# AronCao49/MoPA

Hardware: AMD Instinct MI355X
Metric: scans/sec (joint 2D+3D train step) at 1/2/4/8 MI355X; sparse-conv HBM GB/s (higher is better)
Workload: dtype f32

## Files before the change

mopa_amd/csrc/wino4c9.hip:

```cpp
#include "wino4.h"
#include <stdlib.h>
#include <stdio.h>

typedef float f32x16c __attribute__((ext_vector_type(16)));
typedef float f32x4c __attribute__((ext_vector_type(4)));

#define C9_TM 32
#define C9_CN 64
#define C9_KC 16
#define C9_PITCH 34

struct C9Args {
  const float* in; const float* Uq; const float* bias; float* out; const float* stats;
  int ld_in, ld_out, B, H, W, th, tw, T, Cin, Cout, accumulate, imgs_per_group, bn_c0, nco;
  long long* prof;
};

__device__ __forceinline__ void c9_bt(float d0, float d1, float d2, float d3, float d4, float d5, float& t0, float& t1, float& t2, float& t3,
                                      float& t4, float& t5) {
  t0 = fmaf(4.f, d0, fmaf(-5.f, d2, d4));
  const float p = fmaf(-4.f, d2, d4), q = fmaf(-4.f, d1, d3);
  t1 = p + q;
  t2 = p - q;
  const float r = d4 - d2, s = d3 - d1;
  t3 = fmaf(2.f, s, r);
  t4 = fmaf(-2.f, s, r);
  t5 = fmaf(4.f, d1, fmaf(-5.f, d3, d5));
}

template <bool BN>
__global__ __launch_bounds__(512, 2) void k_wino4_conv9(const C9Args a) {
  __shared__ __attribute__((aligned(16))) float c9_lds[36 * C9_KC * C9_PITCH + 36 * 512];
  float* const Vs = c9_lds;
  float* const Ps = c9_lds + 36 * C9_KC * C9_PITCH;
  const int t = threadIdx.x, lane = t & 63, wv = __builtin_amdgcn_readfirstlane(t >> 6);
  const int nco = a.nco;
  const int grp = blockIdx.x / (8 * nco), r8 = blockIdx.x - grp * 8 * nco;
  const int cob = r8 >> 3, tg = grp * 8 + (r8 & 7);
  const int t0 = tg * C9_TM;
  if (t0 >= a.T) return;
  const int co0 = cob * C9_CN;
  const int H = a.H, W = a.W, tw = a.tw, thw = a.th * a.tw;
#ifdef C9_PROFILE
  long long pt[8] = {0, 0, 0, 0, 0, 0, 0, 0}, tprev = __builtin_readcyclecounter();
#define C9_T(K_) { const long long n_ = __builtin_readcyclecounter(); pt[K_] += n_ - tprev; tprev = n_; }
#else
#define C9_T(K_)
#endif

  const int ts = t >> 4, ch = t & 15;
  const int tile = t0 + ts;
  const bool tv = tile < a.T;
  const int tb = tile / thw, rt = tile - tb * thw, ty = rt / tw, tx = rt - ty * tw;
  const int ab = tv ? tb : 0, ay = tv ? ty : 0, ax = tv ? tx : 0;
  const uint32_t ld4 = (uint32_t)a.ld_in * 4u;
  unsigned okm = 0;
  uint32_t cof[6];
#pragma unroll
  for (int i = 0; i < 6; ++i) {
    okm |= (tv && (unsigned)(4 * ay - 1 + i) < (unsigned)H ? 1u : 0u) << i;
    okm |= ((unsigned)(4 * ax - 1 + i) < (unsigned)W ? 1u : 0u) << (8 + i);
    cof[i] = (uint32_t)min(max(4 * ax - 1 + i, 0), W - 1) * ld4 + (uint32_t)ch * 4u;
  }
  const int abH = ab * H, y0 = 4 * ay - 1;
  const bool interior = __all(tv && ty >= 1 && tx >= 1 && 4 * ty + 4 < H && 4 * tx + 4 < W) != 0;
  const char* __restrict__ inb = reinterpret_cast<const char*>(a.in);
  float* __restrict__ vw = Vs + ch * C9_PITCH + ts;
  float sc = 1.f, sh = 0.f;
  bool bn_ch = false;

  const int l32 = lane & 31, lk = lane >> 5, g = wv & 3, coh = wv >> 2;
  const int pa0 = 3 * (g >> 1), pb0 = 3 * (g & 1);
  const int nci = a.Cin / C9_KC;
  const int64_t pstride = (int64_t)a.Cin * a.Cout;
  const int nco32 = a.Cout / 32;
  const char* __restrict__ ub = reinterpret_cast<const char*>(a.Uq + (int64_t)(pa0 * 6 + pb0) * pstride + (int64_t)(cob * 2 + coh) * 512);
  const uint32_t ul = (uint32_t)lane * 16u;

  f32x16c acc[9];
#pragma unroll
  for (int q = 0; q < 9; ++q)
#pragma unroll
    for (int e = 0; e < 16; ++e) acc[q][e] = 0.f;

  auto row_off = [&](const int i) -> uint32_t { return (uint32_t)((abH + min(max(y0 + i, 0), H - 1)) * W) * ld4; };
  const unsigned ps0 = (unsigned)(uintptr_t)(__attribute__((address_space(3))) void*)&Ps[0] + (unsigned)wv * 256u;
  auto patch_dma = [&](const int n, const uint32_t cb) {
    __builtin_amdgcn_global_load_lds((const __attribute__((address_space(1))) void*)(inb + (row_off(n / 6) + cof[n % 6] + cb)),
                                     (__attribute__((address_space(3))) void*)(uintptr_t)(ps0 + (unsigned)n * 2048u), 4, 0, 0);
  };
  auto patch_bn = [&](int cib) {
    if (BN) {
      const int c_ = cib * C9_KC + ch;
      bn_ch = c_ >= a.bn_c0;
      if (bn_ch) {
        const float* __restrict__ sg = a.stats + (int64_t)((tv ? tb : 0) / a.imgs_per_group) * 4 * (a.Cin - a.bn_c0) + (c_ - a.bn_c0);
        sc = sg[0];
        sh = sg[a.Cin - a.bn_c0];
      }
    }
  };
#pragma unroll
  for (int n = 0; n < 36; ++n) patch_dma(n, 0u);
  patch_bn(0);
  const unsigned vr_b = (unsigned)(uintptr_t)(__attribute__((address_space(3))) void*)&Vs[0] +
                        (unsigned)(((pa0 * 6 + pb0) * C9_KC + lk) * C9_PITCH + l32) * 4u;

  for (int cib = 0; cib < nci; ++cib) {
    C9_T(0)
    {
      __builtin_amdgcn_s_waitcnt(0x0F70);
      float d[36];
#pragma unroll
      for (int n = 0; n < 36; ++n) d[n] = Ps[n * 512 + t];
      if (BN || !interior) {
#pragma unroll
        for (int n = 0; n < 36; ++n) {
          float v = d[n];
          if (BN) {
            const float o = fmaf(v, sc, sh);
            v = bn_ch ? (o > 0.f ? o : o * 0.f) : v;
          }
          d[n] = ((okm >> (n / 6)) & (okm >> (8 + n % 6)) & 1u) ? v : 0.f;
        }
      }
      C9_T(1)
      float m[6][6];
#pragma unroll
      for (int j = 0; j < 6; ++j)
        c9_bt(d[j], d[6 + j], d[12 + j], d[18 + j], d[24 + j], d[30 + j], m[0][j], m[1][j], m[2][j], m[3][j], m[4][j], m[5][j]);
#pragma unroll
      for (int i = 0; i < 6; ++i) {
        float v[6];
        c9_bt(m[i][0], m[i][1], m[i][2], m[i][3], m[i][4], m[i][5], v[0], v[1], v[2], v[3], v[4], v[5]);
#pragma unroll
        for (int j = 0; j < 6; ++j) vw[((i * 6 + j) * C9_KC) * C9_PITCH] = v[j];
      }
    }
    C9_T(2)
    __syncthreads();
    C9_T(3)
    {
      const bool more = cib + 1 < nci;
      const uint32_t cb = (uint32_t)((more ? cib + 1 : cib) * C9_KC) * 4u;
      const char* __restrict__ up = ub + (int64_t)cib * nco32 * 2048;
      f32x4c b0, b1, n0, n1;
#define C9_WLOAD(X0, X1, PTR) \
  asm volatile("global_load_dwordx4 %0, %2, %3\n\tglobal_load_dwordx4 %1, %2, %3 offset:1024" : "=&v"(X0), "=&v"(X1) : "v"(ul), "s"(PTR))
#define C9_WWAIT(N, X0, X1) asm volatile("s_waitcnt vmcnt(" #N ")" : "+v"(X0), "+v"(X1))
      C9_WLOAD(b0, b1, up);
#pragma unroll
      for (int q = 0; q < 9; ++q) {
        if (q + 1 < 9) {
          const char* __restrict__ un = up + (int64_t)(((q + 1) / 3) * 6 + (q + 1) % 3) * pstride * 4;
          if (q & 1) { C9_WLOAD(b0, b1, un); } else { C9_WLOAD(n0, n1, un); }
        }
        float av[8];
#define C9_OFF(KK) "i"((((q / 3) * 6 + q % 3) * C9_KC + 2 * (KK)) * C9_PITCH * 4)
        asm volatile("ds_read_b32 %0, %8 offset:%9\n\tds_read_b32 %1, %8 offset:%10\n\tds_read_b32 %2, %8 offset:%11\n\tds_read_b32 %3, %8 offset:%12\n\t"
                     "ds_read_b32 %4, %8 offset:%13\n\tds_read_b32 %5, %8 offset:%14\n\tds_read_b32 %6, %8 offset:%15\n\tds_read_b32 %7, %8 offset:%16\n\t"
                     "s_waitcnt lgkmcnt(0)"
                     : "=&v"(av[0]), "=&v"(av[1]), "=&v"(av[2]), "=&v"(av[3]), "=&v"(av[4]), "=&v"(av[5]), "=&v"(av[6]), "=&v"(av[7])
                     : "v"(vr_b), C9_OFF(0), C9_OFF(1), C9_OFF(2), C9_OFF(3), C9_OFF(4), C9_OFF(5), C9_OFF(6), C9_OFF(7));
        if (q & 1) {
          if (q == 7) { C9_WWAIT(2, n0, n1); } else { C9_WWAIT(8, n0, n1); }
#pragma unroll
          for (int kk = 0; kk < 4; ++kk) acc[q] = __builtin_amdgcn_mfma_f32_32x32x2f32(av[kk], n0[kk], acc[q], 0, 0, 0);
#pragma unroll
          for (int kk = 0; kk < 4; ++kk) acc[q] = __builtin_amdgcn_mfma_f32_32x32x2f32(av[4 + kk], n1[kk], acc[q], 0, 0, 0);
        } else {
          if (q == 0) { C9_WWAIT(2, b0, b1); } else if (q == 8) { C9_WWAIT(0, b0, b1); } else { C9_WWAIT(8, b0, b1); }
#pragma unroll
          for (int kk = 0; kk < 4; ++kk) acc[q] = __builtin_amdgcn_mfma_f32_32x32x2f32(av[kk], b0[kk], acc[q], 0, 0, 0);
#pragma unroll
          for (int kk = 0; kk < 4; ++kk) acc[q] = __builtin_amdgcn_mfma_f32_32x32x2f32(av[4 + kk], b1[kk], acc[q], 0, 0, 0);
        }
        if (q < 6) {
#pragma unroll
          for (int n = 6 * q; n < 6 * q + 6; ++n) patch_dma(n, cb);
        }
      }
      if (more) patch_bn(cib + 1);
    }
    C9_T(4)
    __builtin_amdgcn_s_barrier();
    C9_T(5)
  }

  constexpr float AT[4][6] = {{1.f, 1.f, 1.f, 1.f, 1.f, 0.f}, {0.f, 1.f, -1.f, 2.f, -2.f, 0.f}, {0.f, 1.f, 1.f, 4.f, 4.f, 0.f},
                              {0.f, 1.f, -1.f, 8.f, -8.f, 1.f}};
  float ar_[4][3];
#pragma unroll
  for (int i = 0; i < 4; ++i)
#pragma unroll
    for (int k = 0; k < 3; ++k) ar_[i][k] = (g >> 1) ? AT[i][3 + k] : AT[i][k];
  __builtin_amdgcn_s_waitcnt(0x0F70);
  __syncthreads();
  float* __restrict__ tsb = c9_lds;
  const int stl = t0 + (t >> 4), sq = (t & 15) * 4;
  const f32x4c bv = a.bias ? *reinterpret_cast<const f32x4c*>(a.bias + co0 + sq) : (f32x4c){0.f, 0.f, 0.f, 0.f};
  const int sb_ = stl / thw, sr_ = stl - sb_ * thw, sty = sr_ / tw, stx = sr_ - sty * tw;
  float* __restrict__ obase = a.out + ((int64_t)(sb_ * H + 4 * sty) * W + 4 * stx) * a.ld_out + co0 + sq;
  for (int i = 0; i < 4; ++i) {
#pragma unroll
    for (int e = 0; e < 16; ++e) {
      const int til = 8 * (e >> 2) + 4 * lk + (e & 3);
#pragma unroll
      for (int b = 0; b < 3; ++b) {
        const float tv_ = fmaf(ar_[i][0], acc[b][e], fmaf(ar_[i][1], acc[3 + b][e], ar_[i][2] * acc[6 + b][e]));
        tsb[(((g >> 1) * 6 + pb0 + b) * C9_TM + til) * C9_CN + coh * 32 + l32] = tv_;
      }
    }
    __syncthreads();
    {
      f32x4c tt[6];
#pragma unroll
      for (int b = 0; b < 6; ++b) {
        const f32x4c u0 = *reinterpret_cast<const f32x4c*>(tsb + (b * C9_TM + (t >> 4)) * C9_CN + sq);
        const f32x4c u1 = *reinterpret_cast<const f32x4c*>(tsb + ((6 + b) * C9_TM + (t >> 4)) * C9_CN + sq);
        tt[b] = u0 + u1;
      }
      if (stl < a.T && 4 * sty + i < H) {
        float* __restrict__ o = obase + (int64_t)i * W * a.ld_out;
#pragma unroll
        for (int j = 0; j < 4; ++j) {
          f32x4c y = bv;
#pragma unroll
          for (int b = 0; b < 6; ++b)
            if (AT[j][b] != 0.f) y += AT[j][b] * tt[b];
          if (4 * stx + j < W) {
            f32x4c* __restrict__ op = reinterpret_cast<f32x4c*>(o + (int64_t)j * a.ld_out);
            *op = a.accumulate ? *op + y : y;
          }
        }
      }
    }
    __syncthreads();
  }
#ifdef C9_PROFILE
  C9_T(6)
  if (blockIdx.x == 100 && t == 0)
    for (int k = 0; k < 8; ++k) a.prof[k] = pt[k];
#endif
}


MOPA_API int mopa_wino4_conv9(const float* in, int32_t ld_in, const float* Uq, const float* bias, float* out, int32_t ld_out, int32_t B, int32_t H,
                              int32_t W, int32_t Cin, int32_t Cout, int32_t accumulate, const float* stats, int32_t n_groups, int32_t bn_c0,
                              void* stream) {
  if (B <= 0 || H <= 0 || W <= 0 || Cin <= 0 || Cout <= 0 || Cin % C9_KC || Cout % C9_CN || ld_in < Cin || ld_out < Cout ||
      ((uintptr_t)Uq & 15) || ((uintptr_t)out & 15) || (ld_out & 3) || ((uintptr_t)bias & 15) || !in || !Uq || !out)
    return MOPA_ERR_ARG;
  if (stats && (n_groups < 1 || B % n_groups || bn_c0 < 0 || bn_c0 >= Cin)) return MOPA_ERR_ARG;
  if ((int64_t)B * H * W * ld_in >= (1ll << 30) || (int64_t)B * H * W * ld_out >= (1ll << 31)) return MOPA_ERR_ARG;
  C9Args a;
  a.in = in; a.Uq = Uq; a.bias = bias; a.out = out; a.stats = stats;
  a.ld_in = ld_in; a.ld_out = ld_out; a.B = B; a.H = H; a.W = W; a.th = (H + 3) / 4; a.tw = (W + 3) / 4;
  const int64_t T = (int64_t)B * a.th * a.tw;
  if (T >= (1 << 30)) return MOPA_ERR_ARG;
  a.T = (int)T; a.Cin = Cin; a.Cout = Cout; a.accumulate = accumulate;
  a.imgs_per_group = stats ? B / n_groups : 1;
  a.bn_c0 = stats ? bn_c0 : 0;
  a.nco = Cout / C9_CN;
  a.prof = nullptr;
  const int64_t ntg = (cdiv64(T, C9_TM) + 7) / 8 * 8;
  const int64_t nblk = ntg * a.nco;
  if (nblk >= (1ll << 31)) return MOPA_ERR_ARG;
#ifdef C9_PROFILE
  static long long* prof = nullptr;
  if (!prof) hipMallocManaged(&prof, 128);
  a.prof = prof;
#endif
  if (stats) k_wino4_conv9<true><<<(unsigned)nblk, 512, 0, (hipStream_t)stream>>>(a);
  else k_wino4_conv9<false><<<(unsigned)nblk, 512, 0, (hipStream_t)stream>>>(a);
  MOPA_CHECK_LAUNCH();
#ifdef C9_PROFILE
  hipStreamSynchronize((hipStream_t)stream);
  {
    const double n_ = Cin / C9_KC;
    printf("[c9 profile] block 100 wave 0, cycles per step: loop head %.0f | patch loads + apply %.0f | transform + lds stores %.0f | barrier %.0f | "
           "multiply %.0f | barrier %.0f | output transform + exchange + store (per item) %.0f   (steps per item %.0f)\n",
           prof[0] / n_, prof[1] / n_, prof[2] / n_, prof[3] / n_, prof[4] / n_, prof[5] / n_, (double)prof[6], n_);
  }
#endif
  return MOPA_OK;
}
```

Before: 424.0.

## Use 16-byte global-to-LDS DMA for Winograd input patches when aligned

Adds a WIDE variant of the F(4x4,3x3) Winograd conv kernel. It loads each input patch with 9 global_load_lds dwordx4 transfers per wave instead of 36 scalar dword ones, with precomputed per-lane gather offsets built via shuffles. The LDS patch layout becomes wave-major to match, and the vmcnt waits and DMA issue points inside the multiply loop are rescheduled for the smaller DMA count. The host picks WIDE when the input is 16-byte aligned and ld_in is a multiple of 4. The aim is fewer memory instructions and better coalescing, at the cost of more template instances and extra address setup.

```diff
diff --git a/mopa_amd/csrc/wino4c9.hip b/mopa_amd/csrc/wino4c9.hip
--- a/mopa_amd/csrc/wino4c9.hip
+++ b/mopa_amd/csrc/wino4c9.hip
@@ -28,7 +28,7 @@
   t5 = fmaf(4.f, d1, fmaf(-5.f, d3, d5));
 }
 
-template <bool BN>
+template <bool BN, bool WIDE>
 __global__ __launch_bounds__(512, 2) void k_wino4_conv9(const C9Args a) {
   __shared__ __attribute__((aligned(16))) float c9_lds[36 * C9_KC * C9_PITCH + 36 * 512];
   float* const Vs = c9_lds;
@@ -43,6 +43,7 @@
   const int H = a.H, W = a.W, tw = a.tw, thw = a.th * a.tw;
 #ifdef C9_PROFILE
   long long pt[8] = {0, 0, 0, 0, 0, 0, 0, 0}, tprev = __builtin_readcyclecounter();
+  const long long tstart = tprev;
 #define C9_T(K_) { const long long n_ = __builtin_readcyclecounter(); pt[K_] += n_ - tprev; tprev = n_; }
 #else
 #define C9_T(K_)
@@ -55,14 +56,23 @@
   const int ab = tv ? tb : 0, ay = tv ? ty : 0, ax = tv ? tx : 0;
   const uint32_t ld4 = (uint32_t)a.ld_in * 4u;
   unsigned okm = 0;
-  uint32_t cof[6];
+  uint32_t cof[WIDE ? 9 : 6];
 #pragma unroll
   for (int i = 0; i < 6; ++i) {
     okm |= (tv && (unsigned)(4 * ay - 1 + i) < (unsigned)H ? 1u : 0u) << i;
     okm |= ((unsigned)(4 * ax - 1 + i) < (unsigned)W ? 1u : 0u) << (8 + i);
-    cof[i] = (uint32_t)min(max(4 * ax - 1 + i, 0), W - 1) * ld4 + (uint32_t)ch * 4u;
+    if (!WIDE) cof[i] = (uint32_t)min(max(4 * ax - 1 + i, 0), W - 1) * ld4 + (uint32_t)ch * 4u;
   }
   const int abH = ab * H, y0 = 4 * ay - 1;
+  if (WIDE) {
+    const int src = ((lane >> 2) & 3) * 16;
+    const int db = __shfl(ab, src), dy = __shfl(ay, src), dx = __shfl(ax, src);
+#pragma unroll
+    for (int k = 0; k < 9; ++k) {
+      const int n = 4 * k + (lane >> 4), i = n / 6, j = n - 6 * i;
+      cof[k] = (uint32_t)((db * H + min(max(4 * dy - 1 + i, 0), H - 1)) * W + min(max(4 * dx - 1 + j, 0), W - 1)) * ld4 + (uint32_t)(lane & 3) * 16u;
+    }
+  }
   const bool interior = __all(tv && ty >= 1 && tx >= 1 && 4 * ty + 4 < H && 4 * tx + 4 < W) != 0;
   const char* __restrict__ inb = reinterpret_cast<const char*>(a.in);
   float* __restrict__ vw = Vs + ch * C9_PITCH + ts;
@@ -84,11 +94,18 @@
     for (int e = 0; e < 16; ++e) acc[q][e] = 0.f;
 
   auto row_off = [&](const int i) -> uint32_t { return (uint32_t)((abH + min(max(y0 + i, 0), H - 1)) * W) * ld4; };
-  const unsigned ps0 = (unsigned)(uintptr_t)(__attribute__((address_space(3))) void*)&Ps[0] + (unsigned)wv * 256u;
+  const unsigned ps0 = (unsigned)(uintptr_t)(__attribute__((address_space(3))) void*)&Ps[0] + (unsigned)wv * 9216u;
+  constexpr int NDMA = WIDE ? 9 : 36;
   auto patch_dma = [&](const int n, const uint32_t cb) {
-    __builtin_amdgcn_global_load_lds((const __attribute__((address_space(1))) void*)(inb + (row_off(n / 6) + cof[n % 6] + cb)),
-                                     (__attribute__((address_space(3))) void*)(uintptr_t)(ps0 + (unsigned)n * 2048u), 4, 0, 0);
+    if (WIDE)
+      __builtin_amdgcn_global_load_lds((const __attribute__((address_space(1))) void*)(inb + (cof[n] + cb)),
+                                       (__attribute__((address_space(3))) void*)(uintptr_t)(ps0 + (unsigned)n * 1024u), 16, 0, 0);
+    else
+      __builtin_amdgcn_global_load_lds((const __attribute__((address_space(1))) void*)(inb + (row_off(n / 6) + cof[n % 6] + cb)),
+                                       (__attribute__((address_space(3))) void*)(uintptr_t)(ps0 + (unsigned)n * 256u), 4, 0, 0);
   };
+  auto dmas_at = [](const int q) constexpr -> int { return WIDE ? (q < 3 ? 2 : q < 6 ? 1 : 0) : (q < 6 ? 6 : 0); };
+  auto dma_first = [](const int q) constexpr -> int { return WIDE ? (q < 3 ? 2 * q : 3 + q) : 6 * q; };
   auto patch_bn = [&](int cib) {
     if (BN) {
       const int c_ = cib * C9_KC + ch;
@@ -101,7 +118,7 @@
     }
   };
 #pragma unroll
-  for (int n = 0; n < 36; ++n) patch_dma(n, 0u);
+  for (int n = 0; n < NDMA; ++n) patch_dma(n, 0u);
   patch_bn(0);
   const unsigned vr_b = (unsigned)(uintptr_t)(__attribute__((address_space(3))) void*)&Vs[0] +
                         (unsigned)(((pa0 * 6 + pb0) * C9_KC + lk) * C9_PITCH + l32) * 4u;
@@ -112,7 +129,7 @@
       __builtin_amdgcn_s_waitcnt(0x0F70);
       float d[36];
 #pragma unroll
-      for (int n = 0; n < 36; ++n) d[n] = Ps[n * 512 + t];
+      for (int n = 0; n < 36; ++n) d[n] = Ps[wv * 2304 + n * 64 + lane];
       if (BN || !interior) {
 #pragma unroll
         for (int n = 0; n < 36; ++n) {
@@ -125,6 +142,9 @@
         }
       }
       C9_T(1)
+#ifdef C9_PROFILE
+      if (cib == 0) pt[7] = tprev - tstart;
+#endif
       float m[6][6];
 #pragma unroll
       for (int j = 0; j < 6; ++j)
@@ -147,7 +167,7 @@
       f32x4c b0, b1, n0, n1;
 #define C9_WLOAD(X0, X1, PTR) \
   asm volatile("global_load_dwordx4 %0, %2, %3\n\tglobal_load_dwordx4 %1, %2, %3 offset:1024" : "=&v"(X0), "=&v"(X1) : "v"(ul), "s"(PTR))
-#define C9_WWAIT(N, X0, X1) asm volatile("s_waitcnt vmcnt(" #N ")" : "+v"(X0), "+v"(X1))
+#define C9_WWAIT(N, X0, X1) asm volatile("s_waitcnt vmcnt(%2)" : "+v"(X0), "+v"(X1) : "i"(N))
       C9_WLOAD(b0, b1, up);
 #pragma unroll
       for (int q = 0; q < 9; ++q) {
@@ -163,22 +183,21 @@
                      : "=&v"(av[0]), "=&v"(av[1]), "=&v"(av[2]), "=&v"(av[3]), "=&v"(av[4]), "=&v"(av[5]), "=&v"(av[6]), "=&v"(av[7])
                      : "v"(vr_b), C9_OFF(0), C9_OFF(1), C9_OFF(2), C9_OFF(3), C9_OFF(4), C9_OFF(5), C9_OFF(6), C9_OFF(7));
         if (q & 1) {
-          if (q == 7) { C9_WWAIT(2, n0, n1); } else { C9_WWAIT(8, n0, n1); }
+          C9_WWAIT(2 + dmas_at(q - 1), n0, n1);
 #pragma unroll
           for (int kk = 0; kk < 4; ++kk) acc[q] = __builtin_amdgcn_mfma_f32_32x32x2f32(av[kk], n0[kk], acc[q], 0, 0, 0);
 #pragma unroll
           for (int kk = 0; kk < 4; ++kk) acc[q] = __builtin_amdgcn_mfma_f32_32x32x2f32(av[4 + kk], n1[kk], acc[q], 0, 0, 0);
         } else {
-          if (q == 0) { C9_WWAIT(2, b0, b1); } else if (q == 8) { C9_WWAIT(0, b0, b1); } else { C9_WWAIT(8, b0, b1); }
+          C9_WWAIT(q == 0 ? 2 : q == 8 ? 0 : 2 + dmas_at(q - 1), b0, b1);
 #pragma unroll
           for (int kk = 0; kk < 4; ++kk) acc[q] = __builtin_amdgcn_mfma_f32_32x32x2f32(av[kk], b0[kk], acc[q], 0, 0, 0);
 #pragma unroll
           for (int kk = 0; kk < 4; ++kk) acc[q] = __builtin_amdgcn_mfma_f32_32x32x2f32(av[4 + kk], b1[kk], acc[q], 0, 0, 0);
         }
-        if (q < 6) {
-#pragma unroll
-          for (int n = 6 * q; n < 6 * q + 6; ++n) patch_dma(n, cb);
-        }
+#pragma unroll
+        for (int k = 0; k < (WIDE ? 2 : 6); ++k)
+          if (k < dmas_at(q)) patch_dma(dma_first(q) + k, cb);
       }
       if (more) patch_bn(cib + 1);
     }
@@ -271,16 +290,23 @@
   if (!prof) hipMallocManaged(&prof, 128);
   a.prof = prof;
 #endif
-  if (stats) k_wino4_conv9<true><<<(unsigned)nblk, 512, 0, (hipStream_t)stream>>>(a);
-  else k_wino4_conv9<false><<<(unsigned)nblk, 512, 0, (hipStream_t)stream>>>(a);
+  const bool wide = !((uintptr_t)in & 15) && !(ld_in & 3);
+  if (stats) {
+    if (wide) k_wino4_conv9<true, true><<<(unsigned)nblk, 512, 0, (hipStream_t)stream>>>(a);
+    else k_wino4_conv9<true, false><<<(unsigned)nblk, 512, 0, (hipStream_t)stream>>>(a);
+  } else {
+    if (wide) k_wino4_conv9<false, true><<<(unsigned)nblk, 512, 0, (hipStream_t)stream>>>(a);
+    else k_wino4_conv9<false, false><<<(unsigned)nblk, 512, 0, (hipStream_t)stream>>>(a);
+  }
   MOPA_CHECK_LAUNCH();
 #ifdef C9_PROFILE
   hipStreamSynchronize((hipStream_t)stream);
   {
     const double n_ = Cin / C9_KC;
     printf("[c9 profile] block 100 wave 0, cycles per step: loop head %.0f | patch loads + apply %.0f | transform + lds stores %.0f | barrier %.0f | "
-           "multiply %.0f | barrier %.0f | output transform + exchange + store (per item) %.0f   (steps per item %.0f)\n",
-           prof[0] / n_, prof[1] / n_, prof[2] / n_, prof[3] / n_, prof[4] / n_, prof[5] / n_, (double)prof[6], n_);
+           "multiply %.0f | barrier %.0f | output transform + exchange + store (per item) %.0f | prologue (per item, in the first "
+           "two) %.0f   (steps per item %.0f)\n",
+           prof[0] / n_, prof[1] / n_, prof[2] / n_, prof[3] / n_, prof[4] / n_, prof[5] / n_, (double)prof[6], (double)prof[7], n_);
   }
 #endif
   return MOPA_OK;
```

Result: no change. 427.6, median of 6 (+0.8%).
